# Gepetto/mpc-interface

Hardware: AMD Instinct MI355X
Metric: QP assemblies/sec (P,q,G,h), biped N=16 batched (higher is better)
Workload: dtype f64; 1 GPU; C2 biped LIPM N=16 no=36 nc=76, per-instance (A,B)/given/aim, K1 on chip; batch_per_gpu=4096, global_batch=4096, streams=2

## Files before the change

include/mpcasm.h:

```cpp
#ifndef MPCASM_H
#define MPCASM_H

#include <stddef.h>
#include <stdint.h>

#ifdef __cplusplus
extern "C" {
#endif

typedef enum mpcasm_status {
  MPCASM_OK = 0,
  MPCASM_ERR_ARG = -1,
  MPCASM_ERR_PLAN = -2,
  MPCASM_ERR_HIP = -3,
  MPCASM_ERR_NODEVICE = -4,
  MPCASM_ERR_LIMIT = -5
} mpcasm_status;

typedef struct mpcasm_plan mpcasm_plan;


int mpcasm_abi_version(void);
int mpcasm_device_count(void);
int mpcasm_last_hip(void);
const char* mpcasm_status_string(int status);
enum { MPCASM_OPT_PATH = 1, MPCASM_OPT_PHASE_MASK = 2, MPCASM_OPT_RESIDENT_PER_CU = 3, MPCASM_OPT_JIT = 4,
       MPCASM_OPT_P_DIRECT = 5, MPCASM_OPT_RESIDENT_GRID = 6, MPCASM_OPT_JIT_FETCH_RUNS = 7 };
int mpcasm_set_option(int option, int value);
int mpcasm_plan_set_option(mpcasm_plan* plan, int option, int value);
int mpcasm_resident_lds_bytes(const int32_t* h_itab, size_t n_itab, const double* h_dtab, size_t n_dtab,
                              int64_t out[2]);
int mpcasm_jit_check(const int32_t* h_itab, size_t n_itab, const double* h_dtab, size_t n_dtab,
                     char* log, size_t log_capacity);
int mpcasm_fetch_segments(const int32_t* h_itab, size_t n_itab, const double* h_dtab, size_t n_dtab,
                          int limit, int32_t* out, size_t capacity, int64_t* n_words);

int mpcasm_plan_prepare(const mpcasm_plan* plan, int batch);
int mpcasm_jit_stats(int64_t out[3]);

int mpcasm_fill_su(const double* d_A, const double* d_B, double* d_S, double* d_U,
                   int batch, int N, int n, int m, int ltv, void* stream);

int mpcasm_plan_create(const int32_t* h_itab, size_t n_itab,
                       const double* h_dtab, size_t n_dtab,
                       mpcasm_plan** out_plan);
int mpcasm_plan_destroy(mpcasm_plan* plan);

int mpcasm_plan_sizes(const mpcasm_plan* plan, int64_t out[8]);

int mpcasm_plan_csc_sizes(const mpcasm_plan* plan, int64_t out[2]);
// ... 255 lines not shown
```

mpc-interface_amd/csrc/capi.hip:

```cpp
#include <hip/hip_runtime.h>
#include <stdint.h>
#include <stdlib.h>
#include <string.h>

#include <algorithm>
#include <atomic>
#include <climits>
#include <cmath>
#include <mutex>
#include <new>
#include <string>
#include <vector>

#include "jit.h"
#include "kernels.h"

using namespace mpcasm;

namespace mpcasm {
Options g_options;
}

struct PlanOptions {
  int path = -1, jit = -1, per_cu = -1, grid = -1;
// ... 319 lines not shown
  PlanDev d;
  const int rc = host_plan(h_itab, n_itab, h_dtab, n_dtab, &d);
  if (rc != MPCASM_OK) return rc;
  if (!d.rs_ok) return MPCASM_ERR_LIMIT;
  std::vector<char> code;
  std::string text;
  const int small = resident_p_direct_for(d, 1), large = resident_p_direct_for(d, 1 << 30);
  int out = MPCASM_OK;
  if (!jit_available()) {
    text = "libhiprtc.so could not be loaded";
    out = MPCASM_ERR_LIMIT;
  } else {
    for (int form : {small, large}) {
      if (form == large && small != large && out != MPCASM_OK) break;
      d.rs_p_direct = form;
      out = jit_code_for(jit_spec_header(d, h_itab, launch_options(nullptr).fetch_runs), false, 0xBF, &code, &text) ? MPCASM_OK : MPCASM_ERR_HIP;
      if (small == large) break;
    }
  }
  if (log && log_capacity) {
    strncpy(log, text.c_str(), log_capacity - 1);
    log[log_capacity - 1] = 0;
  }
  return out;
}

int mpcasm_fetch_segments(const int32_t* h_itab, size_t n_itab, const double* h_dtab, size_t n_dtab,
                          int limit, int32_t* out, size_t capacity, int64_t* n_words) {
  if (tables_missing(h_itab, h_dtab, n_dtab) || !n_words || (capacity && !out) || limit < 0) return MPCASM_ERR_ARG;
  PlanDev d;
  const int rc = host_plan(h_itab, n_itab, h_dtab, n_dtab, &d);
  if (rc != MPCASM_OK) return rc;
  if (!d.rs_ok) return MPCASM_ERR_LIMIT;
  const std::vector<int32_t> words = jit_fetch_plan(d, h_itab, limit);
  *n_words = (int64_t)words.size();
  if (words.size() > capacity) return MPCASM_ERR_LIMIT;
  if (!words.empty()) memcpy(out, words.data(), words.size() * sizeof(int32_t));
  return MPCASM_OK;
}

int mpcasm_jit_stats(int64_t out[3]) {
  if (!out) return MPCASM_ERR_ARG;
  long v[3];
  jit_stats(v);
  out[0] = v[0];
  out[1] = v[1];
  out[2] = v[2];
  return MPCASM_OK;
}

int mpcasm_plan_prepare(const mpcasm_plan* plan, int batch) {
  if (!plan || batch < 0 || !on_plan_device(plan)) return MPCASM_ERR_ARG;
// ... 951 lines not shown
```

mpc-interface_amd/csrc/jit.h:

```cpp
#pragma once
#include <hip/hip_runtime.h>
#include <stdint.h>

#include <string>
#include <vector>

#include "kernels.h"

namespace mpcasm {

std::string jit_spec_header(const PlanDev& d, const int32_t* h_itab, int seg_limit = FS_MAX);
std::vector<int32_t> jit_fetch_plan(const PlanDev& d, const int32_t* h_itab, int seg_limit);
int jit_compile(const std::string& header, std::vector<char>* code, std::string* log,
                bool stamps = false, int phases = 0xBF);
const void* jit_kernel_for(const PlanDev& d, const int32_t* h_itab, int device, int batch,
                           size_t lds_bytes, int jit, int phase_mask, int fetch_runs);
bool jit_code_for(const std::string& header, bool stamps, int phases, std::vector<char>* code,
                  std::string* log, bool distrust_disk = false);
bool jit_available();
void jit_stats(long out[3]);
void jit_forget(const void* itab);
int jit_launch(const void* kernel, const PlanDev& p, const AssembleCall& call);

}
```

mpc-interface_amd/csrc/jit.hip:

```cpp
#include <dlfcn.h>
#include <hip/hip_runtime.h>
#include <stdint.h>
#include <stdio.h>
#include <stdlib.h>
#include <string.h>

#include <sys/stat.h>
#include <sys/types.h>
#include <unistd.h>

#include <atomic>
#include <condition_variable>
#include <iterator>
#include <map>
#include <mutex>
#include <string>
#include <vector>

#include "jit.h"
#include "kernels.h"

namespace mpcasm {

namespace {
// ... 69 lines not shown
  std::vector<int32_t> out;
  if (limit > FS_MAX) limit = FS_MAX;
  for (int kind = 0; kind < 2; ++kind) {
    const int chunks = kind == 0 ? d.rs_ab / 32 : d.rs_nchunk;
    const int32_t* meta = it + (kind == 0 ? d.off_rs_abmeta : d.off_rs_inmeta);
    for (int k = 0; k < chunks; ++k) {
      std::vector<int32_t> segs = jit_fetch_segments(meta + k * 128, 64);
      if ((int)segs.size() > limit * FS_WORDS || (kind == 1 && k >= 32)) segs.clear();
      out.insert(out.end(), {kind, k, (int32_t)(segs.size() / FS_WORDS)});
      out.insert(out.end(), segs.begin(), segs.end());
    }
  }
  return out;
}

std::string jit_spec_header(const PlanDev& d, const int32_t* it, int seg_limit) {
  std::string s = "// generated by libmpcasm (jit.hip) for one plan\n#pragma once\n"
                  "namespace mpcasm {\nnamespace spec {\nstruct PlanConst {\n";
#define MPCASM_X(f, ...) append(s, "  static constexpr int " #f " = %lld;\n", (long long)d.f);
  MPCASM_PLAN_INT_FIELDS(MPCASM_X, MPCASM_X)
#undef MPCASM_X
  append(s, "  static constexpr unsigned rs_src16 = %lldu;\n};\n", (long long)d.rs_src16);
  const int jc = d.rs_jc <= 3 ? 3 : d.rs_jc <= 4 ? 4 : d.rs_jc <= 5 ? 5 : d.rs_jc <= 8 ? 8 : RS_JC_MAX;
  append(s, "constexpr int JC = %lld;\n", jc);
  append(s, "constexpr int NTRIP = %lld;\n", d.rs_ntrip);
  s += "constexpr int TRIPS[NTRIP + 1][8] = {\n";
  const int32_t* tr = it + d.off_rs_trip;
  for (int t = 0; t <= d.rs_ntrip; ++t) {
    s += "  {";
    for (int k = 0; k < RS_TRIP_WORDS; ++k) append(s, k ? ", %lld" : "%lld", tr[t * RS_TRIP_WORDS + k]);
    s += "},\n";
  }
  s += "};\nconstexpr int WTRIP[8][2] = {";
  const int32_t* wt = it + d.off_rs_wtrip;
  for (int w = 0; w < RS_WAVES; ++w) {
    append(s, "{%lld, ", wt[2 * w]);
    append(s, "%lld}, ", wt[2 * w + 1]);
  }
  s += "};\n";
  const std::vector<int32_t> fetch = jit_fetch_plan(d, it, seg_limit);
  for (int kind = 0; kind < 2; ++kind) {
    const int chunks = kind == 0 ? d.rs_ab / 32 : d.rs_nchunk;
    const char* name = kind == 0 ? "AB" : "IMG";
    std::string counts, table;
    long long on_table = 0;
    for (size_t at = 0; at < fetch.size(); at += 3 + fetch[at + 2] * FS_WORDS) {
      if (fetch[at] != kind) continue;
      const int n = fetch[at + 2];
      if (n == 0 && fetch[at + 1] < 32) on_table |= 1ll << fetch[at + 1];
      append(counts, "%lld, ", n);
      table += "  {";
      for (int g = 0; g < FS_MAX; ++g) {
        table += "{";
        for (int w = 0; w < FS_WORDS; ++w) append(table, w ? ", %lld" : "%lld", g < n ? fetch[at + 3 + g * FS_WORDS + w] : 0);
// ... 132 lines not shown
  FILE* f = fopen(tmp.c_str(), "wb");
  if (!f) return;
  const bool ok = fwrite(code.data(), 1, code.size(), f) == code.size();
  fclose(f);
  if (ok && rename(tmp.c_str(), path.c_str()) == 0)
    ++g_stat_disk_writes;
  else
    (void)unlink(tmp.c_str());
}

struct JitKernel {
  hipModule_t module = nullptr;
  hipFunction_t fn = nullptr;
  int per_cu = 0;
  size_t lds = 0;
  bool failed = false;
  bool building = true;
};

std::mutex g_mutex;
std::condition_variable g_built;
std::map<std::pair<int, std::string>, JitKernel*> g_cache;
struct FastKey {
  const void* itab;
  int device, p_direct, phases, fetch_runs;
  bool operator<(const FastKey& o) const {
    if (fetch_runs != o.fetch_runs) return fetch_runs < o.fetch_runs;
    if (itab != o.itab) return itab < o.itab;
    if (device != o.device) return device < o.device;
    if (p_direct != o.p_direct) return p_direct < o.p_direct;
    return phases < o.phases;
  }
};
std::map<FastKey, JitKernel*> g_fast;

}

bool jit_code_for(const std::string& header, bool stamps, int phases, std::vector<char>* code,
                  std::string* log_out, bool distrust_disk) {
  const char* waves = getenv("MPCASM_JIT_WAVES_PER_EU");
  const std::string options = std::string(stamps ? "stamps " : "") + "phases " + std::to_string(phases) +
                              " waves " + (waves ? waves : "4") +
// ... 15 lines not shown
  }
  ++g_stat_compiled;
  if (getenv("MPCASM_JIT_VERBOSE")) fprintf(stderr, "mpcasm: jit: compiled (%zu bytes)\n", code->size());
  if (!path.empty()) disk_write(path, *code);
  return true;
}

namespace {
}

const void* jit_kernel_for(const PlanDev& d, const int32_t* h_itab, int device, int batch,
                           size_t lds_bytes, int jit, int phase_mask, int fetch_runs) {
  if (jit == 2) return nullptr;
  const bool stamps = (phase_mask & 64) != 0;
  const int phases = stamps ? -1 : phase_mask;
  const FastKey fast{d.itab, stamps ? device + 4096 : device, d.rs_p_direct, phases, fetch_runs};
  const bool may_build = jit == 1 || batch >= JIT_MIN_BATCH;
  JitKernel* slot = nullptr;
  bool mine = false;
  std::string header;
  {
    std::unique_lock<std::mutex> lock(g_mutex);
    auto found = g_fast.find(fast);
    if (found != g_fast.end()) {
      slot = found->second;
    } else if (may_build) {
      header = jit_spec_header(d, h_itab, fast.fetch_runs);
      JitKernel*& by_text = g_cache[std::make_pair(fast.device, header + "//" + std::to_string(phases))];
      if (by_text == nullptr) {
        by_text = new JitKernel();
        mine = true;
      }
      slot = by_text;
      g_fast[fast] = slot;
    } else {
      return nullptr;
    }
    if (!mine) {
      if (slot->building && !may_build) return nullptr;
      g_built.wait(lock, [&] { return !slot->building; });
    }
  }
  if (mine) {
    std::vector<char> code;
    hipModule_t module = nullptr;
    hipFunction_t fn = nullptr;
    bool ok = false;
    for (int attempt = 0; attempt < 2 && !ok; ++attempt) {
      code.clear();
      const long hits = g_stat_disk_hits;
      ok = jit_code_for(header, stamps, phases, &code, nullptr, attempt == 1);
      const bool from_disk = g_stat_disk_hits != hits;
      if (ok && (hipModuleLoadData(&module, code.data()) != hipSuccess ||
                 hipModuleGetFunction(&fn, module, "resident_spec_kernel") != hipSuccess)) {
        (void)hipGetLastError();
        if (module) (void)hipModuleUnload(module);
        module = nullptr;
        fn = nullptr;
        ok = false;
        if (!from_disk) break;
      } else if (!ok) {
        break;
      }
    }
    if (ok && hipFuncSetAttribute(reinterpret_cast<const void*>(fn), hipFuncAttributeMaxDynamicSharedMemorySize,
                                  CU_LDS_BYTES) != hipSuccess) {
      (void)hipGetLastError();
      if (hipFuncSetAttribute(reinterpret_cast<const void*>(fn), hipFuncAttributeMaxDynamicSharedMemorySize,
                              RESIDENT_LDS_LIMIT) != hipSuccess) {
        (void)hipGetLastError();
        ok = false;
      }
    }
    {
      std::lock_guard<std::mutex> lock(g_mutex);
      slot->module = module;
      slot->fn = fn;
      slot->failed = !ok;
      slot->building = false;
    }
    g_built.notify_all();
  }
  std::lock_guard<std::mutex> lock(g_mutex);
  if (slot->failed) return nullptr;
  if (slot->lds != lds_bytes) {
    int n = 0;
    if (hipModuleOccupancyMaxActiveBlocksPerMultiprocessor(&n, slot->fn, RS_NT, lds_bytes) != hipSuccess ||
        n < 1) {
      (void)hipGetLastError();
      slot->failed = true;
      return nullptr;
    }
    slot->per_cu = n;
    slot->lds = lds_bytes;
  }
  return slot;
}

bool jit_available() { return rtc().ok; }

void jit_stats(long out[3]) {
  out[0] = g_stat_compiled;
// ... 8 lines not shown
}

int jit_launch(const void* kernel, const PlanDev& p, const AssembleCall& call) {
  const JitKernel* k = static_cast<const JitKernel*>(kernel);
  AssembleCall c = call;
  int per_cu = k->per_cu;
  if (c.opt.per_cu > 0 && c.opt.per_cu < per_cu) per_cu = c.opt.per_cu;
  long grid = (long)c.num_cus * per_cu;
  if (c.opt.grid > 0 && c.opt.grid < grid) grid = c.opt.grid;
  if (grid > c.batch) grid = c.batch;
  const int32_t* itab = p.itab;
  const double* dtab = p.dtab;
  SrcTable s = c.src;
  unsigned long long* stamps = (c.opt.phase_mask & 64) ? static_cast<unsigned long long*>(c.work) : nullptr;
  void* args[] = {&itab, &dtab, &s, &c.params, &c.given, &c.P, &c.q, &c.G, &c.h, &c.batch, &c.opt.phase_mask, &stamps};
  *c.err = hipModuleLaunchKernel(k->fn, (unsigned)grid, 1, 1, RS_NT, 1, 1, (unsigned)k->lds, c.stream,
                                 args, nullptr);
  return *c.err == hipSuccess ? MPCASM_OK : MPCASM_ERR_HIP;
}

}
```

mpc-interface_amd/csrc/kernels.h:

```cpp
#pragma once
#include <hip/hip_runtime.h>
#include <stddef.h>
#include <stdint.h>

#include <atomic>
#include <vector>

#include "../../include/mpcasm.h"
#include "plan_check.h"
#include "plan_dev.h"
#include "plan_tables.h"

namespace mpcasm {

constexpr int CU_LDS_BYTES = 160 * 1024;
hipError_t allow_whole_lds(const void* fn);

int launch_fill_su(const double* A, const double* B, double* S, double* U, int batch, int N, int n,
                   int m, int ltv, hipStream_t stream, hipError_t* err);
struct FillChoice {
  int kernel, arg, generic, pad, spw, lshift, whole_lines, grid;
  size_t lds;
};
int fill_choose(int batch, int N, int n, int m, int ltv, bool aligned16, FillChoice* out);
// ... 139 lines not shown
int launch_ltv_close(int n, int m, int T, int batch, const double* A, long long strideA, const double* B,
                     long long strideB, const double* K, long long strideK, long long stepK, double* Acl,
                     hipStream_t stream, hipError_t* err);
int launch_ltv_augment(int n, int m, int T, int batch, const double* A, long long strideA, const double* B,
                       long long strideB, const double* K, long long strideK, long long stepK, double* At, double* Bt,
                       double* Kt, hipStream_t stream, hipError_t* err);
int launch_ltv_true_inputs(const PlanDev& p, const SrcTable& src, const double* K, long long strideK,
                           const double* given, long long rows, const double* optim, const int32_t* index,
                           double* out, int count, hipStream_t stream, hipError_t* err);
int launch_goal_distance(const double* preview, long long preview_stride, const double* params,
                         long long nparams, const int32_t* terms, int nterms, int ngoals,
                         double* out, int batch, hipStream_t stream, hipError_t* err);
size_t fused_lds_bytes(const PlanDev& p, int nw);
int launch_assemble_fused(const PlanDev& p, const AssembleCall& call, size_t lds_bytes);
size_t resident_lds_bytes(const PlanDev& p);
int resident_choose_p_direct(const PlanDev& p, int option);
int resident_p_direct_for(const PlanDev& p, int batch);
bool resident_inputs_aligned(const PlanDev& p, const SrcTable& src, const double* params,
                             const double* given);
int launch_assemble_resident(const PlanDev& p, const AssembleCall& call, size_t lds_bytes);
int launch_preview_matrices(const PlanDev& p, const SrcTable& src, double* PM, int batch,
                            hipStream_t stream, hipError_t* err);
int launch_box_transform(double* params, long long nparams, int batch, const int32_t* facets,
                         int nfacets, int op, const double* arg, long long arg_stride,
                         hipStream_t stream, hipError_t* err);
int launch_box_transform_ss(double* params, long long nparams, int batch, const int32_t* facets,
                            int nfacets, int op, const double* L, int lrows, int ss_dim,
                            const double* arg, long long arg_stride, hipStream_t stream,
                            hipError_t* err);
int launch_gather(const double* src, long long src_stride, const int32_t* index, int nnz,
// ... 93 lines not shown
```

mpc-interface_amd/csrc/resident.hip:

```cpp
#ifdef __HIPCC_RTC__
using __hip_internal::int32_t;
using __hip_internal::int64_t;
using __hip_internal::uint32_t;
using __hip_internal::uint64_t;
typedef unsigned long uintptr_t;
#else
#include <hip/hip_runtime.h>
#include <stdint.h>
#endif

#include "device_prims.h"
#include "plan_dev.h"
#ifdef MPCASM_SPEC
#include "plan_spec.h"
#endif
#ifndef __HIPCC_RTC__
#include "kernels.h"
#endif

namespace mpcasm {

namespace {

constexpr int NT = RS_NT;
// ... 16 lines not shown
static_assert(GU == RS_GDESC_PIECES && WT == RS_GDESC_THREADS, "descriptor table of G");

template <class PlanT>
__host__ __device__ inline int resident_v_doubles(const PlanT& p) {
  return (p.rs_vrow0 + p.rtot) * p.rs_ldv + 16;
}

struct ResidentLayout {
  int v, pl, ql, dvec, dcoef, dpar, img, ab, streams, ints, total_doubles;
  int ldp;
  int p_direct;
  int i_rr, i_meta, i_wtrip, i_split, i_lti, i_abmeta, i_gdesc, i_gfix, i_rrwin, i_cscp;
};

template <class PlanT>
__host__ __device__ inline ResidentLayout resident_layout(const PlanT& p) {
  ResidentLayout L;
  L.ldp = even_up_i(p.no);
  int o = 0;
  L.v = o;      o += resident_v_doubles(p);
  L.pl = o;
  L.ql = o;     o += L.ldp;
  L.dvec = o;   o += 2 * L.ldp;
  L.dcoef = o;  o += RS_DIAG_MAX * L.ldp;
  L.dpar = o;   o += RS_DIAG_MAX * L.ldp;
  L.img = o;    o += 2 * p.rs_img;
  L.ab = o;     o += 2 * p.rs_ab;
  L.streams = o; o += 2 * (MAX_SOURCES + 3);
  L.ints = o;
  int i = 0;
  L.i_rr = i;    i += p.nc * (p.rr_packed ? RR_COMPACT : RR_WORDS);
  L.i_meta = i;  i += p.rs_nchunk * 64 * 2;
  L.i_abmeta = i; i += p.rs_ab * 2 * 2;
  L.i_gdesc = i;  i += resident_g_mode(p) == 2 ? GU * WT * 2 : (resident_g_mode(p) == 3 ? 2 * p.csc_gnnz : 0);
  L.i_gfix = i;   i += resident_g_mode(p) == 2 && p.rs_ngfix != 0 ? 2 * WT : 0;
  L.i_rrwin = i;  i += p.rs_compact ? p.nc : 0;
  L.i_cscp = i;   i += resident_g_mode(p) == 3 ? p.csc_pnnz : 0;
  L.i_wtrip = i; i += RS_WAVES * 2;
  L.i_split = i; i += p.rs_nsplit;
  L.i_lti = i;   i += p.rs_nlti * RS_LTI_WORDS;
  o += even_up_i(i) / 2;
  L.p_direct = p.rs_p_direct;
  L.pl = o;
  if (!L.p_direct) o += p.no * L.ldp;
  L.total_doubles = o;
  return L;
}

__device__ __forceinline__ void dma16(const void* gsrc, unsigned lds_base) {
  unsigned keep;
// ... 213 lines not shown

template <int I, int N>
__device__ __forceinline__ void spec_trips(TripState& s) {
  if constexpr (I < N) {
    spec_trip<I>(s);
    __builtin_amdgcn_sched_barrier(0);
    spec_trips<I + 1, N>(s);
  }
}
template <int WAVE>
__device__ __forceinline__ void spec_wave_trips(TripState& s) {
  spec_trips<spec::WTRIP[WAVE][0], spec::WTRIP[WAVE][0] + spec::WTRIP[WAVE][1]>(s);
}
#endif

template <int JC, bool STAMPS, bool GEN, class PlanT>
__device__ __forceinline__ void resident_body(
    const PlanT& p, const int32_t* __restrict__ plan_itab, const double* __restrict__ plan_dtab,
    const SrcTable& src, const double* __restrict__ params, const double* __restrict__ given,
    double* __restrict__ P, double* __restrict__ q, double* __restrict__ G,
    double* __restrict__ h, int batch, int phases, unsigned long long* __restrict__ stamps) {
  extern __shared__ __attribute__((aligned(16))) double lds[];
  const int tid = threadIdx.x, lane = tid & 63;
  const int wave = __builtin_amdgcn_readfirstlane(tid >> 6);
  unsigned long long t_acc[8] = {0, 0, 0, 0, 0, 0, 0, 0}, t_prev = 0;
  const unsigned long long t_begin = STAMPS ? __builtin_amdgcn_s_memtime() : 0;
#define SETUP_STAMP(k)                                                                  \
  if (STAMPS && stamps != nullptr && lane == 0)                                         \
    stamps[((size_t)gridDim.x + blockIdx.x) * (NT / 64) * 8 + wave * 8 + (k)] =         \
        __builtin_amdgcn_s_memtime() - t_begin;
  const bool stamping = STAMPS && stamps != nullptr;
#define MPCASM_STAMP(slot)                                         \
  if (STAMPS && stamping) {                                        \
    const unsigned long long t_now = __builtin_amdgcn_s_memtime(); \
    t_acc[slot] += t_now - t_prev;                                 \
    t_prev = t_now;                                                \
  }
  const ResidentLayout L = resident_layout(p);
  const int no = p.no, nc = p.nc, ldv = p.rs_ldv, vd = p.rs_vd, ldp = L.ldp;

  double* V = lds + L.v;
  double* Pl = lds + L.pl;
  double* ql = lds + L.ql;
  double* dvec = lds + L.dvec;
  double2* dcoef = reinterpret_cast<double2*>(lds + L.dcoef);
  int4* dpar = reinterpret_cast<int4*>(lds + L.dpar);
  double* strm = lds + L.streams;
  int* itb = reinterpret_cast<int*>(lds + L.ints);
  int* rr = itb + L.i_rr;
  int2* meta = reinterpret_cast<int2*>(itb + L.i_meta);
  int* wtrip = itb + L.i_wtrip;
  int* split = itb + L.i_split;
  int* lti = itb + L.i_lti;
// ... 124 lines not shown
  constexpr int ZK = 2;
#else
  constexpr int ZK = 0;
#endif
  int v_zb[ZK > 0 ? ZK : 1];
  const int zt0 = tid >= MW * 64 ? tid - MW * 64 : tid + WT;
#pragma unroll
  for (int k = 0; k < ZK; ++k) {
    const int e = zt0 + k * NT;
    v_zb[k] = L.p_direct && e < p.rs_nzblk * 8 ? (plan_itab + p.off_rs_zblk)[e >> 3] : 0;
  }
  int c_sg[JC], c_dst[JC];
  double c_coef[JC];
  auto load_program = [&]() __attribute__((always_inline)) {
    const int4* prog = reinterpret_cast<const int4*>(plan_itab + p.off_rs_prog);
#pragma unroll
    for (int j = 0; j < JC; ++j) {
      const bool have = j < p.rs_jc;
      const int4 w = have ? prog[j * NT + tid] : int4{0, -1, 0, 0};
      c_sg[j] = w.x;
      c_dst[j] = w.y;
      c_coef[j] = __hiloint2double(w.w, w.z);
    }
  };
#ifdef MPCASM_SPEC
  constexpr int FK = JC <= 5 ? 3 : 0;
#else
  constexpr int FK = 0;
#endif
  const int32_t* gix = src.stride[MAX_SOURCES - 1] == -1
                           ? reinterpret_cast<const int32_t*>(src.ptr[MAX_SOURCES - 1]) : nullptr;
  const char* f_base[FK > 0 ? FK : 1];
  int f_stride[FK > 0 ? FK : 1];
// ... 219 lines not shown
        for (int R = ct + CT; R < nc; R += CT) {
          const int32_t* g = trr + R * RR_WORDS;
          reinterpret_cast<int4*>(rr)[R] =
              int4{g[RR_PACKED], g[RR_PACKED + 1], g[RR_CENTER] | (g[RR_CENTER + 1] << 16), g[RR_EXTREME]};
        }
      }
      if (resident_g_mode(p) == 3) {
        const int2* cg = reinterpret_cast<const int2*>(plan_itab + p.off_csc_g);
        for (int i = ct; i < p.csc_gnnz; i += CT) gdesc[i] = cg[i];
        for (int i = ct; i < p.csc_pnnz; i += CT) (itb + L.i_cscp)[i] = (plan_itab + p.off_csc_p)[i];
      }
      if (ct < RS_WAVES * 2) wtrip[ct] = v_wtrip;
      if (ct < p.rs_nsplit) split[ct] = v_split;
      for (int i = ct + CT; i < p.rs_nsplit; i += CT) split[i] = (plan_itab + p.off_rs_split)[i];
    }
    if (own_gd) {
#pragma unroll
      for (int u = 0; u < GU; ++u) gdesc[u * WT + wt_] = v_gd[u];
      if (p.rs_ngfix != 0) gfix[wt_] = v_gfix;
    }
    if (own_diag) {
      dpar[ct] = int4{v_dpar.x, v_dpar.y, v_dpar.z, v_dpar.w};
      dcoef[ct] = double2{v_dcoef.x, v_dcoef.y};
    }
    SETUP_STAMP(3)
    SETUP_STAMP(4)
    SETUP_STAMP(5)
  }
  lds_barrier();
  SETUP_STAMP(6)
  for (int r = tid; r < p.rtot; r += NT) V[(p.rs_vrow0 + r) * ldv + vd + 1] = 1.0;
// ... 89 lines not shown
    MPCASM_STAMP(0)

    auto compose = [&]() {
      if (p.ndiag != 0) {
        int c = tid;
        asm volatile("" : "+v"(c));
        if (c < no) {
          const int4 par = dpar[c];
          const double2 co = dcoef[c];
          const double w0 = prm[par.x], a0 = prm[par.y], w1 = prm[par.z], a1 = prm[par.w];
          dvec[c] = (w0 * co.x) * co.x + (w1 * co.y) * co.y;
          dvec[ldp + c] = w0 * (co.x * (0.0 - a0)) + w1 * (co.y * (0.0 - a1));
        }
      }
      if (phases & 1) {
        double va[JC], vg[JC];
  #pragma unroll
        for (int j = 0; j < JC; ++j) {
          va[j] = img[c_sg[j] & 0xFFFF];
          vg[j] = img[(unsigned)c_sg[j] >> 16];
        }
        double acc = 0.0;
  #pragma unroll
        for (int j = 0; j < JC; ++j) {
          acc += c_coef[j] * va[j] * vg[j];
          if (c_dst[j] >= 0) {
            if (c_dst[j] & RS_DST_ACC)
              __hip_atomic_fetch_add(&V[c_dst[j] & ~RS_DST_ACC], acc, __ATOMIC_RELAXED,
                                     __HIP_MEMORY_SCOPE_WORKGROUP);
            else
              V[c_dst[j]] = acc;
          }
          acc = c_dst[j] >= 0 ? 0.0 : acc;
        }
      }
    };
    const long nxt = instance_at(iter + 1), nxt2 = instance_at(iter + 2);
    if (wave < MW) {
      compose();
      lds_barrier();
      MPCASM_STAMP(1)
      __builtin_amdgcn_s_setprio(2);
      if (lookahead && nxt < batch && (phases & 16)) fetch_image(nxt, buf ^ 1, iter >= 1);
      if (wave == 0 && (GEN && p.rs_nlti != 0) && nxt2 < batch) fetch_ab(nxt2, buf);
      MPCASM_STAMP(7)
      if (wave == MW - 1 && (GEN && p.rs_nlti != 0) && nxt < batch) generate_sources(buf ^ 1, buf ^ 1);
    } else {
      compose();
      lds_barrier();
// ... 27 lines not shown
          double2* G2 = reinterpret_cast<double2*>(Gb);
          int wt_ = wt;
          asm volatile("" : "+v"(wt_));
          const bool all_single = p.rs_gsingle == (1 << (GU * (WT / 64))) - 1;
#ifdef MPCASM_SPEC
          constexpr int GB = spec::PlanConst::rs_gsingle == (1 << (GU * (WT / 64))) - 1 ? GU : 3;
#else
          constexpr int GB = 3;
#endif
          static_assert(GU % GB == 0, "batches of pieces");
          const bool h_mine = wt_ < nc;
          int fix_u = RS_GFIX_NONE;
          double fa1 = 0.0;
          double2 fv1{0.0, 0.0};
          int2 fd{0, 0};
          if (p.rs_ngfix != 0) fd = gfix[wt_];
          const int4 hc4 = reinterpret_cast<const int4*>(rr)[h_mine ? wt_ : 0];
          const int4 hr = int4{0, hc4.w, hc4.x, hc4.y};
          const int2 hc = int2{hc4.z & 0xFFFF, (int)((unsigned)hc4.z >> 16)};
          double ha0 = 0.0, ha1 = 0.0, hc0 = 0.0, hc1 = 0.0, hd0 = 0.0, hd1 = 0.0, hext = 0.0;
#pragma unroll
          for (int u0 = 0; u0 < GU; u0 += GB) {
            int2 ds[GB];
#pragma unroll
            for (int u = 0; u < GB; ++u) ds[u] = gdesc[(u0 + u) * WT + wt_];
            if (u0 == 0 && p.rs_ngfix != 0) {
              fix_u = (unsigned)fd.x >> 16;
              fa1 = prm[fd.y];
              fv1 = *reinterpret_cast<const double2*>(V + (fd.x & 0xFFFF));
            }
            if (u0 == 0) {
              ha0 = prm[hr.w & 0xFFFF];
              ha1 = prm[(unsigned)hr.w >> 16];
              hc0 = prm[hc.x];
              hc1 = prm[hc.y];
              hd0 = V[(hr.z & 0xFFFF) + vd];
              hd1 = V[((unsigned)hr.z >> 16) + vd];
              hext = prm[hr.y];
            }
            double a0[GB], a1[GB];
// ... 381 lines not shown
  const size_t with_p = (size_t)resident_layout(q).total_doubles * sizeof(double);
  q.rs_p_direct = 1;
  const size_t without = (size_t)resident_layout(q).total_doubles * sizeof(double);
  constexpr size_t HALF_CU = 80 * 1024;
  const double per_instance = 8.0 * ((double)p.no * p.no + p.no + (double)p.nc * p.no + p.nc);
  if (with_p > HALF_CU && without <= HALF_CU && per_instance < 128.0 * 1024) return 1;
  return per_instance * batch < 560e6 ? 1 : 0;
}

size_t resident_lds_bytes(const PlanDev& p) {
  if (!p.rs_ok || p.rs_jc > RS_JC_MAX || p.no > WT || p.no < 1 || p.max_axes > AXMAX) return 0;
  if ((long)(p.rs_vrow0 + p.rtot) * p.rs_ldv > (1 << 20)) return 0;
  return (size_t)resident_layout(p).total_doubles * sizeof(double);
}

bool resident_inputs_aligned(const PlanDev& p, const SrcTable& src, const double* params,
                             const double* given) {
  if (p.rs_unit != 16) return true;
  auto ok = [](const void* base, long long stride) {
    return (reinterpret_cast<uintptr_t>(base) & 15) == 0 && (stride & 1) == 0;
  };
  for (int s = 0; s < p.nsrc; ++s)
    if (((p.rs_src16 >> s) & 1) && !ok(src.ptr[s], src.stride[s])) return false;
  return ok(given, p.ng) && ok(params, p.nparams);
}

int launch_assemble_resident(const PlanDev& p, const AssembleCall& call, size_t lds_bytes) {
  if (p.rs_jc <= 3) return launch_jc<3>(p, call, lds_bytes);
  if (p.rs_jc <= 4) return launch_jc<4>(p, call, lds_bytes);
  if (p.rs_jc <= 5) return launch_jc<5>(p, call, lds_bytes);
// ... 7 lines not shown
```

mpc-interface_amd/mpcasm/capi.py:

```python
import ctypes
import os

_HERE = os.path.dirname(os.path.abspath(__file__))
LIB_PATH = os.environ.get("MPCASM_LIB") or os.path.join(_HERE, "libmpcasm.so")

OK = 0
ERR_LIMIT = -5
OPT_PATH = 1
OPT_PHASE_MASK = 2
OPT_RESIDENT_PER_CU = 3
OPT_RESIDENT_GRID = 6
OPT_P_DIRECT = 5
OPT_JIT_FETCH_RUNS = 7
OPT_JIT = 4
PHASE_DEFAULT = 0xBF
PHASE_STAMPS = 0x40
STATUS = {
    0: "MPCASM_OK",
    -1: "MPCASM_ERR_ARG",
    -2: "MPCASM_ERR_PLAN",
    -3: "MPCASM_ERR_HIP",
    -4: "MPCASM_ERR_NODEVICE",
    -5: "MPCASM_ERR_LIMIT",
}
QP_SOLVED, QP_MAX_ITER, QP_PRIMAL_INFEASIBLE, QP_DUAL_INFEASIBLE, QP_NON_CVX = 1, -2, -3, -4, -7
QP_STATUS = {
    1: "MPCASM_QP_SOLVED",
    -2: "MPCASM_QP_MAX_ITER",
    -3: "MPCASM_QP_PRIMAL_INFEASIBLE",
    -4: "MPCASM_QP_DUAL_INFEASIBLE",
    -7: "MPCASM_QP_NON_CVX",
# ... 24 lines not shown
_QP_SOFT = [_void_p, _void_p, ctypes.c_int64]
SIGNATURES = {
    "mpcasm_abi_version": (ctypes.c_int, []),
    "mpcasm_device_count": (ctypes.c_int, []),
    "mpcasm_last_hip": (ctypes.c_int, []),
    "mpcasm_status_string": (ctypes.c_char_p, [ctypes.c_int]),
    "mpcasm_set_option": (ctypes.c_int, [ctypes.c_int, ctypes.c_int]),
    "mpcasm_fill_su": (ctypes.c_int, [_void_p, _void_p, _void_p, _void_p, ctypes.c_int, ctypes.c_int, ctypes.c_int,
                       ctypes.c_int, ctypes.c_int, _void_p]),
    "mpcasm_fill_route": (ctypes.c_int, [ctypes.c_int] * 6 + [_int32_p]),
    "mpcasm_plan_create": (ctypes.c_int, _TABLES + [ctypes.POINTER(_void_p)]),
    "mpcasm_plan_destroy": (ctypes.c_int, [_void_p]),
    "mpcasm_resident_lds_bytes": (ctypes.c_int, _TABLES + [_int64_p]),
    "mpcasm_jit_check": (ctypes.c_int, _TABLES + [ctypes.c_char_p, ctypes.c_size_t]),
    "mpcasm_fetch_segments": (ctypes.c_int, _TABLES + [ctypes.c_int, _void_p, ctypes.c_size_t, _int64_p]),
    "mpcasm_preview_route": (ctypes.c_int, _TABLES + [_int64_p, ctypes.c_int, ctypes.c_int, _int32_p]),
    "mpcasm_sweep_route": (ctypes.c_int, _TABLES + [_int32_p]),
    "mpcasm_tiled_route": (ctypes.c_int, _TABLES + [_int64_p, ctypes.c_int, ctypes.c_int, ctypes.c_int, _int32_p]),
    "mpcasm_assemble_route": (ctypes.c_int, _TABLES + [ctypes.c_int] * 4 + [_int32_p]),
    "mpcasm_staged_route": (ctypes.c_int, _TABLES + [ctypes.c_int] * 3 + [_int32_p]),
    "mpcasm_plan_sizes": (ctypes.c_int, [_void_p, _int64_p]),
    "mpcasm_plan_csc_sizes": (ctypes.c_int, [_void_p, _int64_p]),
    "mpcasm_plan_set_option": (ctypes.c_int, [_void_p, ctypes.c_int, ctypes.c_int]),
    "mpcasm_assemble_indexed": (ctypes.c_int, _PLAN_SRC + [_void_p] * 8 + [ctypes.c_int, _void_p]),
    "mpcasm_plan_last_kernel": (ctypes.c_int, [_void_p]),
    "mpcasm_plan_prepare": (ctypes.c_int, [_void_p, ctypes.c_int]),
    "mpcasm_jit_stats": (ctypes.c_int, [_int64_p]),
    "mpcasm_workspace_bytes": (ctypes.c_int, [_void_p, ctypes.c_int, ctypes.POINTER(ctypes.c_size_t)]),
    "mpcasm_assemble": (ctypes.c_int, _PLAN_SRC + [_void_p] * 7 + [ctypes.c_int, _void_p]),
    "mpcasm_preview_matrices": (ctypes.c_int, _PLAN_SRC + [_void_p, ctypes.c_int, _void_p]),
# ... 129 lines not shown
```

mpc-interface_amd/mpcasm/plan.py:

```python
import collections
import hashlib
from types import SimpleNamespace

import numpy as np
import scipy.sparse as sp

from . import _tables

globals().update({_n: _tables.VALUES[_n] for _n in """
    PLAN_MAGIC PLAN_VERSION H_WORDS MAX_SOURCES SEG_WORDS GT_WORDS LM_WORDS LX_WORDS
    GT_FLAG_P GT_FLAG_HALF GT_FLAG_DIAG
    RS_NW RS_NT RS_WAVES RS_JC_MAX RS_TRIP_WORDS RS_BLOCKS_MAX RS_LTI_WORDS RS_LTI_MAX RS_AXMAX RS_RR_WORDS
    RS_GDESC_PIECES RS_GDESC_THREADS RS_GFIX_NONE RS_DST_ACC RS_DIAG_MAX
    RT_A RT_B RT_D RT_W RT_AIM RT_WORD RT_BI RT_BJ
    RT_SHORT RT_HALF RT_NOP RT_FIRST RT_LAST RT_LIVE RT_QMASK RT_TERM_END
    T_BLOCK T_SID_CONST T_STAGE_WORDS T_LTI_WORDS T_PIG_MAX
    TS_FLAG_P TS_FLAG_HALF TS_FLAG_SIMPLE_A TS_FLAG_SIMPLE_B TS_FLAG_SAME TS_FLAG_G TS_FLAG_TOEPLITZ
    T_SCAN_KMAX T_SCAN_BLKMAX T_SCAN_NMAX T_SCAN_GT_WORDS
    SW_NMAX SW_MMAX SW_AXMAX SW_AXIS_WORDS SW_TERM_WORDS SW_LIM_WORDS SW_LAX_WORDS""".split()})
SEG_GATHER, SEG_IDENTITY = _tables.VALUES["SEG_KIND_GATHER"], _tables.VALUES["SEG_KIND_IDENTITY"]
_H = {_n[2:]: _tables.VALUES[_n] for _n in _tables.ENUMS["HeaderWord"] if _n != "H_WORDS"}

TRIP_COST, TRIP_STEP_COST, TERM_COST, TRIP_Q_COST, PACK_COST, G_PIECE_COST = 200, 30, 60, 60, 250, 500
G_DESC_PIECE_COST = 330
# ... 648 lines not shown
            else:
                pieces.append((0, int(c), i, False))
        heap = [(0, t) for t in range(NT)]
        heapq.heapify(heap)
        trial = [[] for _ in range(NT)]
        for pc in sorted(pieces, key=lambda pc: (pc[0] - pc[1], pc[2], pc[0])):
            load, t = heapq.heappop(heap)
            trial[t].append(pc)
            heapq.heappush(heap, (load + pc[1] - pc[0], t))
        if max((sum(pc[1] - pc[0] for pc in own) for own in trial), default=0) <= cap:
            owner = trial
            split = sorted({ws.index(*divmod(int(fd_idx[pc[2]]), ldv)) for pc in pieces if pc[3]})
            break
    if owner is None:
        return out
    jc = max(1, max((sum(pc[1] - pc[0] for pc in own) for own in owner), default=0))
    src = np.zeros((jc, NT), dtype=np.int32)
    gidx = np.full((jc, NT), image["given"] + ng, dtype=np.int32)
    dst = -np.ones((jc, NT), dtype=np.int32)
    coef = np.zeros((jc, NT))
    for t, own in enumerate(owner):
        j = 0
        for lo, hi, i, shared in sorted(own, key=lambda pc: (pc[2], pc[0])):
            for o in kept[i][lo:hi]:
                src[j, t] = op_img[o]
                gi = (int(ops[o, 1]) >> 16) - 1
                if gi >= 0:
                    gidx[j, t] = image["given"] + gi
                coef[j, t] = pool[int(ops[o, 1]) & 0xFFFF]
                j += 1
# ... 1211 lines not shown
```

Baseline: 180.4 million assemblies/s.

## Specialize compose per wavefront and keep G descriptors in registers

The compose step is now generated per wavefront. Each wave runs only the program slots it actually uses, and waves with no given-operand terms skip the given gather. The host planner reorders thread ownership so that threads with given operands and many slots are grouped into the same waves, which lets the per-wave slot counts shrink. G descriptors and fixups can also be held in registers instead of LDS, which cuts LDS use and may raise occupancy. The JIT builds an LDS fallback and keeps it if the register form spills more scratch. The risks are added register pressure, different rounding where fp contraction is disabled, and extra compile time.

After: 182.0 million assemblies/s (median of 6 runs). Within noise of the previous version (+0.9%).

```diff
diff --git a/include/mpcasm.h b/include/mpcasm.h
--- a/include/mpcasm.h
+++ b/include/mpcasm.h
@@ -34,6 +34,8 @@
                      char* log, size_t log_capacity);
 int mpcasm_fetch_segments(const int32_t* h_itab, size_t n_itab, const double* h_dtab, size_t n_dtab,
                           int limit, int32_t* out, size_t capacity, int64_t* n_words);
+int mpcasm_compose_waves(const int32_t* h_itab, size_t n_itab, const double* h_dtab, size_t n_dtab,
+                         int32_t out[16]);
 
 int mpcasm_plan_prepare(const mpcasm_plan* plan, int batch);
 int mpcasm_jit_stats(int64_t out[3]);
diff --git a/mpc-interface_amd/csrc/capi.hip b/mpc-interface_amd/csrc/capi.hip
--- a/mpc-interface_amd/csrc/capi.hip
+++ b/mpc-interface_amd/csrc/capi.hip
@@ -357,7 +357,8 @@
     for (int form : {small, large}) {
       if (form == large && small != large && out != MPCASM_OK) break;
       d.rs_p_direct = form;
-      out = jit_code_for(jit_spec_header(d, h_itab, launch_options(nullptr).fetch_runs), false, 0xBF, &code, &text) ? MPCASM_OK : MPCASM_ERR_HIP;
+      const LaunchOptions opt = launch_options(nullptr);
+      out = jit_code_for(jit_spec_header(d, h_itab, opt.fetch_runs, jit_switches(opt.phase_mask)), false, 0xBF, &code, &text) ? MPCASM_OK : MPCASM_ERR_HIP;
       if (small == large) break;
     }
   }
@@ -379,6 +380,19 @@
   *n_words = (int64_t)words.size();
   if (words.size() > capacity) return MPCASM_ERR_LIMIT;
   if (!words.empty()) memcpy(out, words.data(), words.size() * sizeof(int32_t));
+  return MPCASM_OK;
+}
+
+int mpcasm_compose_waves(const int32_t* h_itab, size_t n_itab, const double* h_dtab, size_t n_dtab,
+                         int32_t out[16]) {
+  if (tables_missing(h_itab, h_dtab, n_dtab) || !out) return MPCASM_ERR_ARG;
+  PlanDev d;
+  const int rc = host_plan(h_itab, n_itab, h_dtab, n_dtab, &d);
+  if (rc != MPCASM_OK) return rc;
+  if (!d.rs_ok) return MPCASM_ERR_LIMIT;
+  const std::vector<int32_t> words = jit_compose_waves(d, h_itab);
+  static_assert(RS_WAVES * 2 == 16, "mpcasm.h: out[16]");
+  memcpy(out, words.data(), words.size() * sizeof(int32_t));
   return MPCASM_OK;
 }
 
diff --git a/mpc-interface_amd/csrc/jit.h b/mpc-interface_amd/csrc/jit.h
--- a/mpc-interface_amd/csrc/jit.h
+++ b/mpc-interface_amd/csrc/jit.h
@@ -9,8 +9,12 @@
 
 namespace mpcasm {
 
-std::string jit_spec_header(const PlanDev& d, const int32_t* h_itab, int seg_limit = FS_MAX);
+constexpr int JIT_COMPOSE_BY_WAVE = 1, JIT_GDESC_IN_REGS = 2;
+int jit_switches(int phase_mask);
+std::string jit_spec_header(const PlanDev& d, const int32_t* h_itab, int seg_limit = FS_MAX,
+                            int switches = JIT_COMPOSE_BY_WAVE | JIT_GDESC_IN_REGS);
 std::vector<int32_t> jit_fetch_plan(const PlanDev& d, const int32_t* h_itab, int seg_limit);
+std::vector<int32_t> jit_compose_waves(const PlanDev& d, const int32_t* h_itab);
 int jit_compile(const std::string& header, std::vector<char>* code, std::string* log,
                 bool stamps = false, int phases = 0xBF);
 const void* jit_kernel_for(const PlanDev& d, const int32_t* h_itab, int device, int batch,
diff --git a/mpc-interface_amd/csrc/jit.hip b/mpc-interface_amd/csrc/jit.hip
--- a/mpc-interface_amd/csrc/jit.hip
+++ b/mpc-interface_amd/csrc/jit.hip
@@ -107,7 +107,30 @@
   return out;
 }
 
-std::string jit_spec_header(const PlanDev& d, const int32_t* it, int seg_limit) {
+std::vector<int32_t> jit_compose_waves(const PlanDev& d, const int32_t* it) {
+  std::vector<int32_t> out(RS_WAVES * 2, 0);
+  const int32_t* prog = it + d.off_rs_prog;
+  const int one = d.rs_img_given + d.ng;
+  for (int t = 0; t < RS_NT; ++t) {
+    int slots = 0;
+    for (int j = 0; j < d.rs_jc; ++j)
+      if (prog[(j * RS_NT + t) * 4 + 1] >= 0) slots = j + 1;
+    bool given = false;
+    for (int j = 0; j < slots; ++j)
+      given = given || (int)((uint32_t)prog[(j * RS_NT + t) * 4] >> 16) != one;
+    int32_t* w = &out[(t / 64) * 2];
+    if (slots > w[0]) w[0] = slots;
+    if (given) w[1] = 1;
+  }
+  return out;
+}
+
+int jit_switches(int phase_mask) {
+  const char* off = getenv("MPCASM_JIT_SWITCHES_OFF");
+  return (JIT_COMPOSE_BY_WAVE | JIT_GDESC_IN_REGS) & ~(phase_mask >> 15) & ~(off ? atoi(off) : 0);
+}
+
+std::string jit_spec_header(const PlanDev& d, const int32_t* it, int seg_limit, int switches) {
   std::string s = "// generated by libmpcasm (jit.hip) for one plan\n#pragma once\n"
                   "namespace mpcasm {\nnamespace spec {\nstruct PlanConst {\n";
 #define MPCASM_X(f, ...) append(s, "  static constexpr int " #f " = %lld;\n", (long long)d.f);
@@ -131,6 +154,19 @@
     append(s, "%lld}, ", wt[2 * w + 1]);
   }
   s += "};\n";
+  const std::vector<int32_t> cw = jit_compose_waves(d, it);
+  std::string slots, given;
+  long long packed = 0;
+  for (int w = 0; w < RS_WAVES; ++w) {
+    append(slots, "%lld, ", cw[2 * w]);
+    append(given, "%lld, ", cw[2 * w + 1]);
+    packed |= (long long)cw[2 * w] << (4 * w);
+  }
+  static_assert(RS_JC_MAX < 16 && RS_WAVES * 4 <= 32, "CWAVE_SLOTS_PACKED");
+  s += "constexpr int CWAVE_SLOTS[8] = {" + slots + "};\nconstexpr int CWAVE_GIVEN[8] = {" + given + "};\n";
+  append(s, "constexpr unsigned CWAVE_SLOTS_PACKED = %lldu;\n", packed);
+  append(s, "constexpr bool COMPOSE_BY_WAVE = %lld;\n", (switches & JIT_COMPOSE_BY_WAVE) != 0);
+  append(s, "constexpr bool GDESC_IN_REGS = %lld;\n", (switches & JIT_GDESC_IN_REGS) != 0);
   const std::vector<int32_t> fetch = jit_fetch_plan(d, it, seg_limit);
   for (int kind = 0; kind < 2; ++kind) {
     const int chunks = kind == 0 ? d.rs_ab / 32 : d.rs_nchunk;
@@ -293,6 +329,8 @@
   hipFunction_t fn = nullptr;
   int per_cu = 0;
   size_t lds = 0;
+  size_t lds_gd_regs = 0;
+  bool gd_regs = false;
   bool failed = false;
   bool building = true;
 };
@@ -302,9 +340,10 @@
 std::map<std::pair<int, std::string>, JitKernel*> g_cache;
 struct FastKey {
   const void* itab;
-  int device, p_direct, phases, fetch_runs;
+  int device, p_direct, phases, fetch_runs, switches;
   bool operator<(const FastKey& o) const {
     if (fetch_runs != o.fetch_runs) return fetch_runs < o.fetch_runs;
+    if (switches != o.switches) return switches < o.switches;
     if (itab != o.itab) return itab < o.itab;
     if (device != o.device) return device < o.device;
     if (p_direct != o.p_direct) return p_direct < o.p_direct;
@@ -350,7 +389,8 @@
   if (jit == 2) return nullptr;
   const bool stamps = (phase_mask & 64) != 0;
   const int phases = stamps ? -1 : phase_mask;
-  const FastKey fast{d.itab, stamps ? device + 4096 : device, d.rs_p_direct, phases, fetch_runs};
+  const FastKey fast{d.itab, stamps ? device + 4096 : device, d.rs_p_direct, phases, fetch_runs,
+                     jit_switches(phase_mask)};
   const bool may_build = jit == 1 || batch >= JIT_MIN_BATCH;
   JitKernel* slot = nullptr;
   bool mine = false;
@@ -361,7 +401,7 @@
     if (found != g_fast.end()) {
       slot = found->second;
     } else if (may_build) {
-      header = jit_spec_header(d, h_itab, fast.fetch_runs);
+      header = jit_spec_header(d, h_itab, fast.fetch_runs, fast.switches);
       JitKernel*& by_text = g_cache[std::make_pair(fast.device, header + "//" + std::to_string(phases))];
       if (by_text == nullptr) {
         by_text = new JitKernel();
@@ -378,25 +418,50 @@
     }
   }
   if (mine) {
-    std::vector<char> code;
     hipModule_t module = nullptr;
     hipFunction_t fn = nullptr;
-    bool ok = false;
-    for (int attempt = 0; attempt < 2 && !ok; ++attempt) {
-      code.clear();
-      const long hits = g_stat_disk_hits;
-      ok = jit_code_for(header, stamps, phases, &code, nullptr, attempt == 1);
-      const bool from_disk = g_stat_disk_hits != hits;
-      if (ok && (hipModuleLoadData(&module, code.data()) != hipSuccess ||
-                 hipModuleGetFunction(&fn, module, "resident_spec_kernel") != hipSuccess)) {
+    const auto build = [&](const std::string& text, hipModule_t* mod, hipFunction_t* f) {
+      std::vector<char> code;
+      bool ok = false;
+      for (int attempt = 0; attempt < 2 && !ok; ++attempt) {
+        code.clear();
+        const long hits = g_stat_disk_hits;
+        ok = jit_code_for(text, stamps, phases, &code, nullptr, attempt == 1);
+        const bool from_disk = g_stat_disk_hits != hits;
+        if (ok && (hipModuleLoadData(mod, code.data()) != hipSuccess ||
+                   hipModuleGetFunction(f, *mod, "resident_spec_kernel") != hipSuccess)) {
+          (void)hipGetLastError();
+          if (*mod) (void)hipModuleUnload(*mod);
+          *mod = nullptr;
+          *f = nullptr;
+          ok = false;
+          if (!from_disk) break;
+        } else if (!ok) {
+          break;
+        }
+      }
+      return ok;
+    };
+    const auto scratch_bytes = [](hipFunction_t f) {
+      int bytes = 0;
+      if (hipFuncGetAttribute(&bytes, HIP_FUNC_ATTRIBUTE_LOCAL_SIZE_BYTES, f) != hipSuccess) {
         (void)hipGetLastError();
-        if (module) (void)hipModuleUnload(module);
-        module = nullptr;
-        fn = nullptr;
-        ok = false;
-        if (!from_disk) break;
-      } else if (!ok) {
-        break;
+        return 1 << 30;
+      }
+      return bytes;
+    };
+    bool ok = build(header, &module, &fn);
+    bool gd_regs = ok && (fast.switches & JIT_GDESC_IN_REGS) && resident_lds_bytes_gd_regs(d) != lds_bytes;
+    if (gd_regs && scratch_bytes(fn) > 0) {
+      hipModule_t module2 = nullptr;
+      hipFunction_t fn2 = nullptr;
+      if (build(jit_spec_header(d, h_itab, fast.fetch_runs, fast.switches & ~JIT_GDESC_IN_REGS), &module2, &fn2)) {
+        if (scratch_bytes(fn) > scratch_bytes(fn2)) {
+          (void)hipModuleUnload(module);
+          module = module2, fn = fn2, gd_regs = false;
+        } else {
+          (void)hipModuleUnload(module2);
+        }
       }
     }
     if (ok && hipFuncSetAttribute(reinterpret_cast<const void*>(fn), hipFuncAttributeMaxDynamicSharedMemorySize,
@@ -412,6 +477,8 @@
       std::lock_guard<std::mutex> lock(g_mutex);
       slot->module = module;
       slot->fn = fn;
+      slot->gd_regs = gd_regs;
+      slot->lds_gd_regs = gd_regs ? resident_lds_bytes_gd_regs(d) : 0;
       slot->failed = !ok;
       slot->building = false;
     }
@@ -421,7 +488,8 @@
   if (slot->failed) return nullptr;
   if (slot->lds != lds_bytes) {
     int n = 0;
-    if (hipModuleOccupancyMaxActiveBlocksPerMultiprocessor(&n, slot->fn, RS_NT, lds_bytes) != hipSuccess ||
+    if (hipModuleOccupancyMaxActiveBlocksPerMultiprocessor(&n, slot->fn, RS_NT,
+                                                           slot->gd_regs ? slot->lds_gd_regs : lds_bytes) != hipSuccess ||
         n < 1) {
       (void)hipGetLastError();
       slot->failed = true;
@@ -460,7 +528,8 @@
   SrcTable s = c.src;
   unsigned long long* stamps = (c.opt.phase_mask & 64) ? static_cast<unsigned long long*>(c.work) : nullptr;
   void* args[] = {&itab, &dtab, &s, &c.params, &c.given, &c.P, &c.q, &c.G, &c.h, &c.batch, &c.opt.phase_mask, &stamps};
-  *c.err = hipModuleLaunchKernel(k->fn, (unsigned)grid, 1, 1, RS_NT, 1, 1, (unsigned)k->lds, c.stream,
+  *c.err = hipModuleLaunchKernel(k->fn, (unsigned)grid, 1, 1, RS_NT, 1, 1,
+                                 (unsigned)(k->gd_regs ? k->lds_gd_regs : k->lds), c.stream,
                                  args, nullptr);
   return *c.err == hipSuccess ? MPCASM_OK : MPCASM_ERR_HIP;
 }
diff --git a/mpc-interface_amd/csrc/kernels.h b/mpc-interface_amd/csrc/kernels.h
--- a/mpc-interface_amd/csrc/kernels.h
+++ b/mpc-interface_amd/csrc/kernels.h
@@ -177,6 +177,7 @@
 size_t fused_lds_bytes(const PlanDev& p, int nw);
 int launch_assemble_fused(const PlanDev& p, const AssembleCall& call, size_t lds_bytes);
 size_t resident_lds_bytes(const PlanDev& p);
+size_t resident_lds_bytes_gd_regs(const PlanDev& p);
 int resident_choose_p_direct(const PlanDev& p, int option);
 int resident_p_direct_for(const PlanDev& p, int batch);
 bool resident_inputs_aligned(const PlanDev& p, const SrcTable& src, const double* params,
diff --git a/mpc-interface_amd/csrc/resident.hip b/mpc-interface_amd/csrc/resident.hip
--- a/mpc-interface_amd/csrc/resident.hip
+++ b/mpc-interface_amd/csrc/resident.hip
@@ -54,7 +54,7 @@
 };
 
 template <class PlanT>
-__host__ __device__ inline ResidentLayout resident_layout(const PlanT& p) {
+__host__ __device__ inline ResidentLayout resident_layout(const PlanT& p, bool gd_regs = false) {
   ResidentLayout L;
   L.ldp = even_up_i(p.no);
   int o = 0;
@@ -72,8 +72,8 @@
   L.i_rr = i;    i += p.nc * (p.rr_packed ? RR_COMPACT : RR_WORDS);
   L.i_meta = i;  i += p.rs_nchunk * 64 * 2;
   L.i_abmeta = i; i += p.rs_ab * 2 * 2;
-  L.i_gdesc = i;  i += resident_g_mode(p) == 2 ? GU * WT * 2 : (resident_g_mode(p) == 3 ? 2 * p.csc_gnnz : 0);
-  L.i_gfix = i;   i += resident_g_mode(p) == 2 && p.rs_ngfix != 0 ? 2 * WT : 0;
+  L.i_gdesc = i;  i += resident_g_mode(p) == 2 ? (gd_regs ? 0 : GU * WT * 2) : (resident_g_mode(p) == 3 ? 2 * p.csc_gnnz : 0);
+  L.i_gfix = i;   i += resident_g_mode(p) == 2 && p.rs_ngfix != 0 && !gd_regs ? 2 * WT : 0;
   L.i_rrwin = i;  i += p.rs_compact ? p.nc : 0;
   L.i_cscp = i;   i += resident_g_mode(p) == 3 ? p.csc_pnnz : 0;
   L.i_wtrip = i; i += RS_WAVES * 2;
@@ -317,6 +317,51 @@
 }
 #endif
 
+__device__ __forceinline__ double mul_then_add(double c, double a, double acc) {
+#pragma clang fp contract(off)
+  const double t = c * a;
+  return acc + t;
+}
+template <int S, bool GIVEN, int JC>
+__device__ __forceinline__ void compose_slots(const double* img, double* V, const int (&c_sg)[JC],
+                                              const int (&c_dst)[JC], const double (&c_coef)[JC]) {
+  static_assert(S <= JC, "slots of the program");
+  double va[S > 0 ? S : 1], vg[S > 0 ? S : 1];
+#pragma unroll
+  for (int j = 0; j < S; ++j) {
+    va[j] = img[c_sg[j] & 0xFFFF];
+    if (GIVEN) vg[j] = img[(unsigned)c_sg[j] >> 16];
+  }
+  double acc = 0.0;
+#pragma unroll
+  for (int j = 0; j < S; ++j) {
+    if (GIVEN)
+      acc += c_coef[j] * va[j] * vg[j];
+    else
+      acc = mul_then_add(c_coef[j], va[j], acc);
+    if (c_dst[j] >= 0) {
+      if (c_dst[j] & RS_DST_ACC)
+        __hip_atomic_fetch_add(&V[c_dst[j] & ~RS_DST_ACC], acc, __ATOMIC_RELAXED, __HIP_MEMORY_SCOPE_WORKGROUP);
+      else
+        V[c_dst[j]] = acc;
+    }
+    acc = c_dst[j] >= 0 ? 0.0 : acc;
+  }
+}
+#ifdef MPCASM_SPEC
+__device__ __forceinline__ int spec_wave_slots(int wave) {
+  return spec::COMPOSE_BY_WAVE ? (int)((spec::CWAVE_SLOTS_PACKED >> (4 * wave)) & 15u) : spec::JC;
+}
+template <int W>
+__device__ __forceinline__ void spec_wave_compose(const double* img, double* V, const int (&c_sg)[spec::JC],
+                                                  const int (&c_dst)[spec::JC], const double (&c_coef)[spec::JC]) {
+  if constexpr (spec::COMPOSE_BY_WAVE)
+    compose_slots<spec::CWAVE_SLOTS[W], spec::CWAVE_GIVEN[W] != 0>(img, V, c_sg, c_dst, c_coef);
+  else
+    compose_slots<spec::JC, true>(img, V, c_sg, c_dst, c_coef);
+}
+#endif
+
 template <int JC, bool STAMPS, bool GEN, class PlanT>
 __device__ __forceinline__ void resident_body(
     const PlanT& p, const int32_t* __restrict__ plan_itab, const double* __restrict__ plan_dtab,
@@ -339,7 +384,17 @@
     t_acc[slot] += t_now - t_prev;                                 \
     t_prev = t_now;                                                \
   }
-  const ResidentLayout L = resident_layout(p);
+#ifdef MPCASM_SPEC
+  constexpr bool GD_REGS = spec::GDESC_IN_REGS && PlanT::csc_gnnz == 0 && PlanT::csc_pnnz == 0 &&
+                           PlanT::rr_packed != 0 && PlanT::rs_ngdesc != 0;
+  constexpr bool GD_PACK = GD_REGS && PlanT::rs_gsingle == (1 << (GU * (WT / 64))) - 1;
+#else
+  constexpr bool GD_REGS = false, GD_PACK = false;
+#endif
+  int2 r_gd[GD_REGS ? GU : 1], r_gfix = int2{0, 0};
+#pragma unroll
+  for (int u = 0; u < (GD_REGS ? GU : 1); ++u) r_gd[u] = int2{0, 0};
+  const ResidentLayout L = resident_layout(p, GD_REGS);
   const int no = p.no, nc = p.nc, ldv = p.rs_ldv, vd = p.rs_vd, ldp = L.ldp;
 
   double* V = lds + L.v;
@@ -494,9 +549,14 @@
   double c_coef[JC];
   auto load_program = [&]() __attribute__((always_inline)) {
     const int4* prog = reinterpret_cast<const int4*>(plan_itab + p.off_rs_prog);
+#ifdef MPCASM_SPEC
+    const int slots = spec_wave_slots(wave);
+#else
+    const int slots = JC;
+#endif
 #pragma unroll
     for (int j = 0; j < JC; ++j) {
-      const bool have = j < p.rs_jc;
+      const bool have = j < p.rs_jc && j < slots;
       const int4 w = have ? prog[j * NT + tid] : int4{0, -1, 0, 0};
       c_sg[j] = w.x;
       c_dst[j] = w.y;
@@ -746,7 +806,12 @@
       if (ct < p.rs_nsplit) split[ct] = v_split;
       for (int i = ct + CT; i < p.rs_nsplit; i += CT) split[i] = (plan_itab + p.off_rs_split)[i];
     }
-    if (own_gd) {
+    if (own_gd && GD_REGS) {
+#pragma unroll
+      for (int u = 0; u < (GD_REGS ? GU : 1); ++u)
+        r_gd[u] = GD_PACK ? int2{(v_gd[u].x & 0xFFFF) | (v_gd[u].y << 16), 0} : v_gd[u];
+      r_gfix = v_gfix;
+    } else if (own_gd) {
 #pragma unroll
       for (int u = 0; u < GU; ++u) gdesc[u * WT + wt_] = v_gd[u];
       if (p.rs_ngfix != 0) gfix[wt_] = v_gfix;
@@ -866,25 +931,23 @@
         }
       }
       if (phases & 1) {
-        double va[JC], vg[JC];
-  #pragma unroll
-        for (int j = 0; j < JC; ++j) {
-          va[j] = img[c_sg[j] & 0xFFFF];
-          vg[j] = img[(unsigned)c_sg[j] >> 16];
-        }
-        double acc = 0.0;
-  #pragma unroll
-        for (int j = 0; j < JC; ++j) {
-          acc += c_coef[j] * va[j] * vg[j];
-          if (c_dst[j] >= 0) {
-            if (c_dst[j] & RS_DST_ACC)
-              __hip_atomic_fetch_add(&V[c_dst[j] & ~RS_DST_ACC], acc, __ATOMIC_RELAXED,
-                                     __HIP_MEMORY_SCOPE_WORKGROUP);
-            else
-              V[c_dst[j]] = acc;
-          }
-          acc = c_dst[j] >= 0 ? 0.0 : acc;
-        }
+#ifdef MPCASM_SPEC
+        static_assert(RS_WAVES == 8, "one case per wavefront");
+        if (!spec::COMPOSE_BY_WAVE) {
+          compose_slots<JC, true>(img, V, c_sg, c_dst, c_coef);
+        } else switch (wave) {
+          case 0: spec_wave_compose<0>(img, V, c_sg, c_dst, c_coef); break;
+          case 1: spec_wave_compose<1>(img, V, c_sg, c_dst, c_coef); break;
+          case 2: spec_wave_compose<2>(img, V, c_sg, c_dst, c_coef); break;
+          case 3: spec_wave_compose<3>(img, V, c_sg, c_dst, c_coef); break;
+          case 4: spec_wave_compose<4>(img, V, c_sg, c_dst, c_coef); break;
+          case 5: spec_wave_compose<5>(img, V, c_sg, c_dst, c_coef); break;
+          case 6: spec_wave_compose<6>(img, V, c_sg, c_dst, c_coef); break;
+          default: spec_wave_compose<7>(img, V, c_sg, c_dst, c_coef); break;
+        }
+#else
+        compose_slots<JC, true>(img, V, c_sg, c_dst, c_coef);
+#endif
       }
     };
     const long nxt = instance_at(iter + 1), nxt2 = instance_at(iter + 2);
@@ -942,7 +1005,7 @@
           double fa1 = 0.0;
           double2 fv1{0.0, 0.0};
           int2 fd{0, 0};
-          if (p.rs_ngfix != 0) fd = gfix[wt_];
+          if (p.rs_ngfix != 0) fd = GD_REGS ? r_gfix : gfix[wt_];
           const int4 hc4 = reinterpret_cast<const int4*>(rr)[h_mine ? wt_ : 0];
           const int4 hr = int4{0, hc4.w, hc4.x, hc4.y};
           const int2 hc = int2{hc4.z & 0xFFFF, (int)((unsigned)hc4.z >> 16)};
@@ -951,7 +1014,12 @@
           for (int u0 = 0; u0 < GU; u0 += GB) {
             int2 ds[GB];
 #pragma unroll
-            for (int u = 0; u < GB; ++u) ds[u] = gdesc[(u0 + u) * WT + wt_];
+            for (int u = 0; u < GB; ++u) {
+              int2 r = r_gd[GD_REGS ? u0 + u : 0];
+              if (GD_REGS) asm volatile("" : "+v"(r.x));
+              if (GD_REGS && !GD_PACK) asm volatile("" : "+v"(r.y));
+              ds[u] = GD_PACK ? int2{r.x, (int)((unsigned)r.x >> 16)} : (GD_REGS ? r : gdesc[(u0 + u) * WT + wt_]);
+            }
             if (u0 == 0 && p.rs_ngfix != 0) {
               fix_u = (unsigned)fd.x >> 16;
               fa1 = prm[fd.y];
@@ -1363,6 +1431,11 @@
   return (size_t)resident_layout(p).total_doubles * sizeof(double);
 }
 
+size_t resident_lds_bytes_gd_regs(const PlanDev& p) {
+  if (resident_lds_bytes(p) == 0) return 0;
+  return (size_t)resident_layout(p, true).total_doubles * sizeof(double);
+}
+
 bool resident_inputs_aligned(const PlanDev& p, const SrcTable& src, const double* params,
                              const double* given) {
   if (p.rs_unit != 16) return true;
diff --git a/mpc-interface_amd/mpcasm/capi.py b/mpc-interface_amd/mpcasm/capi.py
--- a/mpc-interface_amd/mpcasm/capi.py
+++ b/mpc-interface_amd/mpcasm/capi.py
@@ -15,6 +15,8 @@
 OPT_JIT = 4
 PHASE_DEFAULT = 0xBF
 PHASE_STAMPS = 0x40
+PHASE_COMPOSE_ALL_SLOTS = 1 << 15
+PHASE_GDESC_IN_LDS = 1 << 16
 STATUS = {
     0: "MPCASM_OK",
     -1: "MPCASM_ERR_ARG",
@@ -69,6 +71,7 @@
     "mpcasm_resident_lds_bytes": (ctypes.c_int, _TABLES + [_int64_p]),
     "mpcasm_jit_check": (ctypes.c_int, _TABLES + [ctypes.c_char_p, ctypes.c_size_t]),
     "mpcasm_fetch_segments": (ctypes.c_int, _TABLES + [ctypes.c_int, _void_p, ctypes.c_size_t, _int64_p]),
+    "mpcasm_compose_waves": (ctypes.c_int, _TABLES + [_void_p]),
     "mpcasm_preview_route": (ctypes.c_int, _TABLES + [_int64_p, ctypes.c_int, ctypes.c_int, _int32_p]),
     "mpcasm_sweep_route": (ctypes.c_int, _TABLES + [_int32_p]),
     "mpcasm_tiled_route": (ctypes.c_int, _TABLES + [_int64_p, ctypes.c_int, ctypes.c_int, ctypes.c_int, _int32_p]),
diff --git a/mpc-interface_amd/mpcasm/plan.py b/mpc-interface_amd/mpcasm/plan.py
--- a/mpc-interface_amd/mpcasm/plan.py
+++ b/mpc-interface_amd/mpcasm/plan.py
@@ -686,6 +686,15 @@
             break
     if owner is None:
         return out
+    def _given_op(own):
+        return any((int(ops[o, 1]) >> 16) != 0 for lo, hi, i, _ in own for o in kept[i][lo:hi])
+
+    if _os.environ.get("MPCASM_COMPOSE_ORDER") != "0":
+        ranked = sorted(range(NT), key=lambda t: (not _given_op(owner[t]), -sum(pc[1] - pc[0] for pc in owner[t]), t))
+        placed = [None] * NT
+        for k, t in enumerate(ranked):
+            placed[(k + NW * 64) % NT] = owner[t]
+        owner = placed
     jc = max(1, max((sum(pc[1] - pc[0] for pc in own) for own in owner), default=0))
     src = np.zeros((jc, NT), dtype=np.int32)
     gidx = np.full((jc, NT), image["given"] + ng, dtype=np.int32)
```
